# fusiyuan2010/CSC

Measured on AMD Instinct MI355X. Metric: encode MB/s (10^6 input bytes / wall-clock) on enwik9 stand-in, -m3 -d64m; stream bit-exact vs reference, higher is better.
Workload: dtype u8/u32 (byte + 32-bit integer work; 12-bit probabilities, 64-bit range-coder low)

## Files before the change

### csc_amd/csrc/csc_kernels.hip

```cpp
#include <hip/hip_runtime.h>
#include <stdint.h>
#include <stdlib.h>

#include "csc_device.h"
#include "csc_tables.h"

namespace cscmi {

#define DEV __device__ __forceinline__
#define GLOBAL_AS __attribute__((address_space(1)))
typedef GLOBAL_AS uint8_t gu8;
typedef GLOBAL_AS uint16_t gu16;
typedef GLOBAL_AS uint32_t gu32;
typedef uint32_t __attribute__((ext_vector_type(4))) raw_vec4;
typedef GLOBAL_AS raw_vec4 gvec4;
#define UNI(x) ((uint32_t)__builtin_amdgcn_readfirstlane((int)(x)))

#ifndef CSCMI_TU
#define CSCMI_TU 0
#endif
static __device__ __constant__ uint32_t d_p2bits[512];
static __device__ __constant__ uint32_t d_logtable[513];

__device__ static const uint32_t kDltIndex[5] = {1, 2, 3, 4, 8};
// ... 113 lines not shown
    c.ht2 = uni_gptr(c.ht2); c.ht3 = uni_gptr(c.ht3); c.ht6 = uni_gptr(c.ht6); c.bt_head = uni_gptr(c.bt_head); c.bt_nodes = uni_gptr(c.bt_nodes);
    c.p_lit = uni_gptr(c.p_lit); c.p_delta = uni_gptr(c.p_delta); c.mfbuf = uni_gptr(c.mfbuf);
    c.ht6_off = UNI(c.ht6_off); c.bth_off = UNI(c.bth_off);
    c.ht_bits = UNI(c.ht_bits); c.ht_width = UNI(c.ht_width); c.ht_low = UNI(c.ht_low); c.ht_cyc = UNI(c.ht_cyc);
    c.bt_bits = UNI(c.bt_bits); c.bt_size = UNI(c.bt_size); c.bt_cyc = UNI(c.bt_cyc); c.good_len = UNI(c.good_len);
    c.lz_good_len = UNI(c.lz_good_len); c.lz_bt_cyc = UNI(c.lz_bt_cyc); c.lz_ht_cyc = UNI(c.lz_ht_cyc);
    c.bt_pos = UNI(c.bt_pos); c.pos = UNI(c.pos); c.wnd_curpos = UNI(c.wnd_curpos);
    c.state = UNI(c.state); c.ctx = UNI(c.ctx); c.lp_rebuild_int = UNI(c.lp_rebuild_int);
    c.rc_low = uni64(c.rc_low); c.rc_range = UNI(c.rc_range); c.rc_cache = UNI(c.rc_cache); c.rc_cachesize = UNI(c.rc_cachesize);
    c.rc_size = UNI(c.rc_size); c.bc_size = UNI(c.bc_size); c.bc_curbits = UNI(c.bc_curbits); c.bc_curval = UNI(c.bc_curval); c.bsize = UNI(c.bsize);
    c.rc_buf = uni_gptr(c.rc_buf); c.bc_buf = uni_gptr(c.bc_buf); c.arena = uni_gptr(c.arena); c.swapbuf = uni_gptr(c.swapbuf);
    c.arena_used = UNI(c.arena_used); c.arena_cap = UNI(c.arena_cap); c.error = UNI(c.error);
    c.stage_base = UNI(c.stage_base); c.stage_end = UNI(c.stage_end);
    c.wv = UNI(c.wv); c.dp_seq = UNI(c.dp_seq); c.dp_idle = UNI(c.dp_idle); c.dp_seq_seen = UNI(c.dp_seq_seen);
    c.st_find = UNI(c.st_find); c.st_slide = UNI(c.st_slide); c.st_bt = UNI(c.st_bt); c.st_lit = UNI(c.st_lit); c.st_match = UNI(c.st_match);
    c.q_head = UNI(c.q_head); c.q_room = UNI(c.q_room);
}

DEV void wave_fence() { __builtin_amdgcn_fence(__ATOMIC_SEQ_CST, "workgroup"); }
DEV uint32_t rdlane(uint32_t v, uint32_t lane) { return (uint32_t)__builtin_amdgcn_readlane((int)v, (int)lane); }
DEV uint32_t wrlane(uint32_t val, uint32_t lane, uint32_t old) { return (threadIdx.x & 63u) == lane ? val : old; }

DEV uint64_t load8u(const gu8 *p)
{
    uintptr_t a = (uintptr_t)p;
    uint32_t sh = (uint32_t)a & 3u;
    const gu32 *q = (const gu32 *)(a & ~(uintptr_t)3);
    uint32_t d0 = q[0], d1 = q[1], d2 = q[2];
    uint32_t lo = __builtin_amdgcn_alignbyte(d1, d0, sh);
    uint32_t hi = __builtin_amdgcn_alignbyte(d2, d1, sh);
    return ((uint64_t)hi << 32) | lo;
}
DEV uint32_t ldb(const gu8 *p) { return UNI((uint32_t)*p); }

DEV uint64_t stage_load8(const uint32_t *stage, uint32_t byte_idx)
{
    uint32_t sh = byte_idx & 3u;
    const uint32_t *q = stage + (byte_idx >> 2);
    uint32_t d0 = q[0], d1 = q[1], d2 = q[2];
    uint32_t lo = __builtin_amdgcn_alignbyte(d1, d0, sh);
    uint32_t hi = __builtin_amdgcn_alignbyte(d2, d1, sh);
    return ((uint64_t)hi << 32) | lo;
}


__device__ __noinline__ void lanes_copy16(gvec4 *d4, const gvec4 *s4, uint32_t n16)
{
    for (uint32_t i = threadIdx.x & 63u; i < n16; i += 64) d4[i] = s4[i];
}
__device__ __noinline__ void lanes_copy8(gu8 *dst, const gu8 *src, uint32_t n)
{
    for (uint32_t t = threadIdx.x & 63u; t < n; t += 64) dst[t] = src[t];
}
__device__ __noinline__ void lanes_fill32(gu32 *dst, uint32_t n, uint32_t v)
{
    for (uint32_t t = threadIdx.x & 63u; t < n; t += 64) dst[t] = v;
}
__device__ __noinline__ void lanes_stage(uint8_t *sb, const gu8 *src, uint32_t first, uint32_t end)
{
    for (uint32_t t = first + (threadIdx.x & 63u); t < end; t += 64) sb[t] = src[t];
}
DEV void emit_block(Sc &c, uint32_t kind, const gu8 *buf, uint32_t size)
{
    uint32_t need = 16 + ((size + 15) & ~15u);
    if (c.arena_used + need > c.arena_cap) { c.error = ERR_ARENA_FULL; return; }
    gu8 *dst = c.arena + c.arena_used;
    wave_fence();
    ((gu32 *)dst)[0] = kind; ((gu32 *)dst)[1] = size;
    lanes_copy16((gvec4 *)(dst + 16), (const gvec4 *)buf, (size + 15) >> 4);
    c.arena_used += need;
}

constexpr uint32_t kCoderQ = 4096;
constexpr uint32_t kPDumpE = P_COUNT + 3;
struct CoderQ {
    uint32_t pub, tail, done, pad;
    uint32_t e[kCoderQ];
};
DEV void q_publish(Sc &c)
{
    __builtin_amdgcn_fence(__ATOMIC_RELEASE, "workgroup", "local");
    *(volatile __attribute__((address_space(3))) uint32_t *)&c.Q->pub = c.q_head;
}
constexpr uint32_t ERR_QUEUE_STALL = 0x40200000u;
DEV uint32_t q_wait_room(Sc &c, uint32_t need)
{
    uint32_t used, spins = 0;
    if (__builtin_expect(c.error != 0, 0)) return 0;
    while ((used = c.q_head - UNI(*(volatile __attribute__((address_space(3))) uint32_t *)&c.Q->tail)) > kCoderQ - need) {
        __builtin_amdgcn_s_sleep(2);
        if (++spins > (1u << 24)) { if (!c.error) c.error = ERR_QUEUE_STALL | (used & 0xFFFFu); return 0; }
    }
    return used;
}
DEV void q_push(Sc &c, uint32_t e)
{
    if (__builtin_expect(c.q_room == 0, 0)) {
        q_publish(c);
        c.q_room = umin(kCoderQ - 64u - q_wait_room(c, 128u), 256u);
    }
    c.Q->e[c.q_head & (kCoderQ - 1)] = e;
    c.q_head++; c.q_room--;
}

DEV void q_push_bits(Sc &c, uint32_t pold, uint32_t bit, uint32_t n, uint32_t from = 0)
{
    if (__builtin_expect(c.q_room < n, 0)) {
        q_publish(c);
        c.q_room = umin(kCoderQ - 64u - q_wait_room(c, 128u), 256u);
    }
    const uint32_t k = c.lane - from;
    c.Q->e[(c.q_head + (k < n ? k : 63u)) & (kCoderQ - 1)] = 0x80000000u | (bit ? 0x1000u : 0u) | pold;
    c.q_head += n; c.q_room -= n;
}

DEV void rc_put(Sc &c, uint32_t byte)
{
    c.rc_buf[c.rc_size++] = (uint8_t)byte;
    if (c.rc_size == c.bsize) { emit_block(c, 1, c.rc_buf, c.bsize); c.rc_size = 0; }
}

DEV void rc_shift_low(Sc &c)
{
    uint32_t low32 = (uint32_t)c.rc_low, top = (uint32_t)(c.rc_low >> 32);
    if (low32 < 0xFF000000u || top != 0) {
        uint32_t temp = c.rc_cache;
        do {
            rc_put(c, (temp + top) & 0xFF);
            temp = 0xFF;
        } while (--c.rc_cachesize != 0);
        c.rc_cache = low32 >> 24;
    }
    c.rc_cachesize++;
    c.rc_low = (uint64_t)(low32 << 8);
}

DEV void rc_code(Sc &c, uint32_t v, uint32_t p)
{
    if (c.Q) { q_push(c, 0x80000000u | (v ? 0x1000u : 0u) | p); return; }
    const uint32_t bound = (c.rc_range >> 12) * p;
    c.rc_low += v ? 0u : bound;
    c.rc_range = v ? bound : c.rc_range - bound;
    if (__builtin_expect(c.rc_range < (1u << 24), 0)) { c.rc_range <<= 8; rc_shift_low(c); }
}
DEV uint32_t p_update(uint32_t v, uint32_t p) { return v ? p + ((0xFFFu - p) >> 5) : p - (p >> 5); }

DEV void enc_bit_lds(Sc &c, uint32_t v, uint32_t idx)
{
    uint32_t p = UNI(c.L->P[idx]);
    c.L->P[idx] = p_update(v, p);
    rc_code(c, v, p);
}

DEV void bc_put(Sc &c, uint32_t byte)
{
    c.bc_buf[c.bc_size++] = (uint8_t)byte;
    if (c.bc_size == c.bsize) { emit_block(c, 0, c.bc_buf, c.bsize); c.bc_size = 0; }
}

DEV void enc_direct16(Sc &c, uint32_t val, uint32_t len)
{
    if (c.Q) { q_push(c, 0x40000000u | (len << 16) | (val & 0xFFFFu)); return; }
    c.bc_curval = (c.bc_curval << len) | val;
    c.bc_curbits += len;
    while (c.bc_curbits >= 8) {
        bc_put(c, (c.bc_curval >> (c.bc_curbits - 8)) & 0xFF);
// ... 412 lines not shown
```

### csc_amd/csrc/csc_kernels_dp4.inc

```

constexpr uint32_t kD4Rec = 256;
constexpr uint32_t kD4CandEnt = kD4Rec * 4;
constexpr uint32_t kD4RefEnt = 256;
constexpr uint32_t kD4Ent = kD4CandEnt + kD4RefEnt;
constexpr uint32_t kD4LA = 48;
constexpr uint32_t kD4Waves = 12;
DEV uint32_t d4_role(uint32_t w)
{
    constexpr uint32_t roles[12] = { 0, 6, 7, 1, 8, 5, 4, 2, 8, 8, 9, 3 };
    return w < 12 ? roles[w] : 8u;
}
constexpr uint32_t kD4Requested = 0xFFFFFFFFu;
#ifndef D4_IDLE_MUL
#define D4_IDLE_MUL 1
#endif
constexpr int kD4IdleSleep = 4 * D4_IDLE_MUL;
constexpr uint32_t kD4RefreshAt = 32;
constexpr uint32_t kD4MaxGood = 16;
constexpr uint32_t kD6Ring = 128;
constexpr uint32_t kD6MRing = 64;
constexpr uint32_t kD4MultiMax = 768;

struct Dp4X {
    uint32_t sb_seq, sb_ack, quit, abort;
    uint32_t sb0, pos0, size, gen;
    uint32_t m_pos;
    uint32_t m_ids[2];
    uint32_t ins_head;
    uint32_t cmp_next, cmp_pause, cmp_idle[3], cmp_cur[3];
    uint32_t ev_seq, ev_s, ev_len, ev_ack;
    uint32_t ref_head;
    uint32_t rq_head, rq_tail;
    uint32_t lit_req, lit_from, lit_done;
    uint32_t rid[4];
    uint32_t io_w0, io_gen, io_state0, io_lp_int, io_lit_seq, io_rq_head, io_wnd_lo, io_wnd_hi, io_wnd_size, io_vld, io_good, io_plit_lo, io_plit_hi;
    alignas(16) uint32_t o_kind, o_end, o_a0l, o_a0code, o_a0eid, o_a0slot, o_fin_i0, o_fin_i1, o_lp_int, o_lit_seq, o_rq_head, o_err;
#ifdef CSCMI_TIMERS
    uint32_t stat[8];
    uint32_t wtm[48];
#endif
    uint32_t rq[16][2];
    raw_vec4 cand[kD4Rec];
    uint8_t hflag[kD4Rec];
    uint32_t rec_tag[kD4Rec], rec_hsum[kD4Rec], rec_a0d[kD4Rec], rec_len[kD4Rec][16];
    uint32_t rec_m32[kD4Rec][16];
    raw_vec4 ent[kD4Ent];
    uint32_t fwd[kD4Ent];
    alignas(512) uint16_t litp[4][kD4Rec];
    alignas(16) uint16_t tab[64][32];
    alignas(256) raw_vec4 lab[16];
    alignas(512) uint32_t tent[2][16][8];
    alignas(256) raw_vec4 ver[16];
    uint32_t lab_seq, win_seq;
    alignas(16) uint32_t dump[8];
    alignas(8) uint32_t e_prog[2]; uint32_t e_stop[2];
#ifdef CSCMI_TIMERS
    uint32_t dbgp[64], dbgq[64][8], dbgl[32];
    uint32_t dbg;
    uint32_t tr_win, tr_lo, tr_hi;
#endif
    uint32_t lenp_new[32];
    uint32_t lt_pub, lt_done;
    uint32_t lt_rec[kD6Ring];
    uint32_t mt_pub, mt_done;
    uint32_t mt_rec[kD6MRing][2];
    uint32_t hS[2], h_reset, hand[20];
};
struct EncLds4 { EncLds base; Dp4X x; CoderQ q; };
__shared__ EncLds4 g_lds4;

DEV uint32_t d4_tag(uint32_t gen, uint32_t p) { return ((gen << 13) | p) + 1u; }
DEV Dp4X *d4x(Sc &c) { return reinterpret_cast<Dp4X *>(c.X); }

DEV uint32_t d4_eq4(uint32_t x)
{
    const uint32_t z = ~(((x & 0x7F7F7F7Fu) + 0x7F7F7F7Fu) | x) & 0x80808080u;
    return (((z >> 7) * 0x01020408u) >> 24) & 0xFu;
}
DEV uint32_t d4_eq8(uint64_t x) { return d4_eq4((uint32_t)x) | (d4_eq4((uint32_t)(x >> 32)) << 4); }

DEV bool d4_spin(Sc &c, Dp4X *X, uint32_t &spins, uint32_t site)
{
    __builtin_amdgcn_s_sleep(1);
    if ((++spins & 1023u) == 0 && (spins > (kDpSpinLimit << 2) || lds_vload(&X->abort))) {
        if (!lds_vload(&X->abort)) lds_vstore(&X->abort, 0x40000000u | (site << 16) | (c.wv << 24) | (spins & 0xFFFFu));
        c.error = lds_vload(&X->abort);
        return false;
    }
    return true;
}
template <int LANE> DEV uint32_t d4_wrlane(uint32_t old, uint32_t val)
{
    asm volatile("v_writelane_b32 %0, %1, %2" : "+v"(old) : "s"(val), "n"(LANE));
    return old;
}
DEV uint32_t umax_(uint32_t a, uint32_t b) { return a > b ? a : b; }
DEV uint32_t d4_parse_pos(Dp4X *X, uint32_t *ids0 = nullptr, uint32_t *ids1 = nullptr)
{
    typedef volatile __attribute__((address_space(3))) uint32_t vu32;
    typedef volatile __attribute__((address_space(3))) raw_vec4 vvec4;
    const uint32_t sq = UNI(*(vu32 *)&X->lab_seq);
    const uint32_t w0 = UNI(*(vu32 *)&X->io_w0), mp = UNI(*(vu32 *)&X->m_pos);
    const bool open = sq - 1u < 0xFFFFFFFEu;
    if (ids0) {
        const raw_vec4 lb = *(vvec4 *)&X->lab[(sq - 1u) & 15u];
        const uint32_t m0 = UNI(*(vu32 *)&X->m_ids[0]), m1 = UNI(*(vu32 *)&X->m_ids[1]);
        *ids0 = open ? UNI(lb.z) : m0; *ids1 = open ? UNI(lb.w) : m1;
    }
    return open ? umax_(mp, w0 + (sq < 2u ? 0u : sq - 2u)) : mp;
}
DEV uint32_t d4_rol1(uint32_t v) { return (uint32_t)__builtin_amdgcn_update_dpp(0, (int)v, 0x134, 0xF, 0xF, false); }


DEV void d4_insert_batch(Sc &c, Dp4X *X, uint32_t i0, uint32_t n, uint32_t &carry_h6)
{
    EncLds *L = c.L;
    const uint32_t lane = c.lane;
    const bool act = lane < n;
    const uint32_t sb0 = c.stage_base;
    const uint64_t v = stage_load8(L->stage, i0 + lane + 16);
    const uint32_t lo = (uint32_t)v, hi = (uint32_t)(v >> 32);
    const uint32_t h2 = hash2_of(lo), h3 = hash3_of(lo), h6 = hash6_mul(lo, hi) >> (32 - c.ht_bits);
// ... 1560 lines not shown
                L->fin2[k * 2u] = cD; L->fin2[k * 2u + 1u] = cBS;
#ifdef CSCMI_TIMERS
                if (k < 64) { X->dbgq[k][0] = cP; X->dbgq[k][5] = eP; X->dbgq[k][6] = 2; X->dbgq[k][7] = lp_int; }
#endif
                lds_fence();
                *(lds_vu32 *)&X->lab_seq = k + 1u;
            }
            vP = cP | vz; vD = cD | vz; vBS = cBS | vz; vI0 = cI0 | vz; vI1 = cI1 | vz; v_lp = lp_int | vz; v_reach = reach | vz;
            fI0 = cI0; fI1 = cI1;
            if (!out) pf_label();
#ifdef CSCMI_TIMERS
            t_gen += __builtin_readcyclecounter() - tg0;
#endif
            if (out) break;
        }
    }
#ifdef CSCMI_TIMERS
    const unsigned long long tse = __builtin_readcyclecounter();
    if (lane == 0) { atomicAdd(&X->wtm[13], (uint32_t)(tse - ts0) >> 4); atomicAdd(&X->wtm[14], n_straight); atomicAdd(&X->wtm[15], 1u);
        atomicAdd(&X->wtm[24], (uint32_t)(ts0 - tsp) >> 4); atomicAdd(&X->wtm[25], (uint32_t)t_first >> 4); atomicAdd(&X->wtm[26], (uint32_t)t_poll >> 4);
        atomicAdd(&X->wtm[27], (uint32_t)t_gen >> 4); atomicAdd(&X->wtm[28], n_gen); atomicAdd(&X->wtm[29], (uint32_t)(tse - t_last) >> 4); }
#endif
    lds_fence();
    *(lds_vu32 *)&X->lab_seq = kD5Stop;
    if (refreshed) { if (lane < 32) L->len_price[lane] = X->lenp_new[lane]; lds_fence(); }
    uint32_t f0 = kind == DP_EXIT_LIMIT ? fI0 : UNI(X->lab[end & 15u].z);
    uint32_t f1 = kind == DP_EXIT_LIMIT ? fI1 : UNI(X->lab[end & 15u].w);
    d5_forward_ids(X, lane, sel_rid, f0, f1);
    *(lds_vu32 *)&X->m_pos = w0 + end; *(lds_vu32 *)&X->m_ids[0] = f0; *(lds_vu32 *)&X->m_ids[1] = f1;
    {
        raw_vec4 o0, o1, o2;
        o0.x = kind; o0.y = end; o0.z = a0l; o0.w = a0code; o1.x = a0eid; o1.y = a0slot; o1.z = f0; o1.w = f1;
        o2.x = v_lp; o2.y = lit_seq; o2.z = rq_head; o2.w = err;
        *(lds_vvec4 *)&X->o_kind = o0; *(lds_vvec4 *)&X->o_a0eid = o1; *(lds_vvec4 *)&X->o_lp_int = o2;
    }
    lds_fence();
#ifdef CSCMI_TIMERS
    if (lane == 0) atomicAdd(&X->wtm[30], (uint32_t)(__builtin_readcyclecounter() - tse) >> 4);
#endif
}

DEV void d4_request(Sc &c, Dp4X *X, uint32_t id, uint32_t base, uint32_t &rq_head)
{
    if (rq_head - lds_vload(&X->rq_tail) >= 16u) return;
    X->rq[rq_head & 15u][0] = id;
    X->rq[rq_head & 15u][1] = base;
    X->fwd[id] = kD4Requested;
    rq_head++;
    lds_fence();
    lds_vstore(&X->rq_head, rq_head);
}

DEV bool d4_rebase_reps(Sc &c, Dp4X *X, uint32_t base, uint32_t &rq_head, bool wait)
{
    for (uint32_t r = 0; r < 4; r++) {
        const uint32_t id = lds_vload(&X->rid[r]);
        const uint32_t f = lds_vload(&X->fwd[id]);
        if (f == 0) {
            uint32_t spins = 0;
            while (rq_head - lds_vload(&X->rq_tail) >= 16u) if (!d4_spin(c, X, spins, 3)) return false;
            d4_request(c, X, id, base, rq_head);
        }
    }
    if (!wait) return true;
    for (uint32_t r = 0; r < 4; r++) {
        uint32_t id = lds_vload(&X->rid[r]);
        uint32_t spins = 0, f;
        while ((f = lds_vload(&X->fwd[id])) == kD4Requested) if (!d4_spin(c, X, spins, 4)) return false;
        if (f) { lds_fence(); X->rid[r] = f - 1; }
    }
    return true;
}


struct D6Cur { uint32_t lt_head, lt_seen, mt_head, mt_seen; };
DEV bool d6_join(Sc &c, Dp4X *X, D6Cur &q, bool lit_only = false);
DEV bool d6_room(Sc &c, Dp4X *X, uint32_t need, D6Cur &q)
{
    if (__builtin_expect(c.q_room < need, 0)) {
#ifdef CSCMI_TIMERS
        const uint64_t t0 = __builtin_readcyclecounter();
        const uint32_t out0 = (q.lt_head - lds_vload(&X->lt_done)) + (q.mt_head - lds_vload(&X->mt_done));
#endif
        if (!d6_join(c, X, q)) return false;
#ifdef CSCMI_TIMERS
        const uint64_t t1 = __builtin_readcyclecounter();
#endif
        q_publish(c);
        c.q_room = kCoderQ - 64u - q_wait_room(c, 64u + need);
#ifdef CSCMI_TIMERS
        if (c.lane == 0) { atomicAdd(&X->wtm[40], 1u); atomicAdd(&X->wtm[41], (uint32_t)(t1 - t0) >> 4); atomicAdd(&X->wtm[42], (uint32_t)(__builtin_readcyclecounter() - t1) >> 4); atomicAdd(&X->wtm[46], c.q_room >> 4);
                           atomicAdd(&X->wtm[31], out0); if (t1 - t0 < 2048u) atomicAdd(&X->wtm[47], 1u); }
#endif
    }
    return true;
}
DEV bool d6_literal(Sc &c, Dp4X *X, uint32_t sym, D6Cur &q)
{
    if (__builtin_expect(q.lt_head - q.lt_seen >= kD6Ring - 8u, 0)) {
        uint32_t spins = 0;
        while (q.lt_head - (q.lt_seen = lds_vload(&X->lt_done)) >= kD6Ring - 8u) if (!d4_spin(c, X, spins, 12)) return false;
    }
    const uint32_t fidx = P_STATE + c.state * 3;
    const uint32_t pold = c.L->P[fidx];
    c.L->P[fidx] = p_update(0, pold);
    c.Q->e[c.q_head & (kCoderQ - 1)] = 0x80000000u | pold;
    *(lds_vu32 *)&X->lt_rec[q.lt_head & (kD6Ring - 1)] = c.ctx | (sym << 8) | (c.q_head << 16);
    q.lt_head++;
    *(lds_vu32 *)&X->lt_pub = q.lt_head;
    c.q_head += 9; c.q_room -= 9;
    c.state = (c.state * 4) & 0x3F;
    c.ctx = sym;
    c.st_lit++;
    return true;
}
DEV void d6_flags(Sc &c, uint32_t nf, uint32_t idx, uint32_t bit)
{
    const bool on = c.lane < nf;
    const uint32_t i = on ? idx : kPDumpE;
    const uint32_t p = c.L->P[i];
    c.L->P[i] = p + (uint32_t)((int32_t)((bit ? 0xFFFu : 31u) - p) >> 5);
    c.Q->e[(c.q_head + (on ? c.lane : 63u)) & (kCoderQ - 1)] = 0x80000000u | (bit << 12) | p;
    c.q_head += nf; c.q_room -= nf;
}
DEV uint32_t d6_len_slots(uint32_t len) { return len < 8 ? 4u : len < 16 ? 5u : 9u; }
DEV bool d6_tree_record(Sc &c, Dp4X *X, uint32_t w0, uint32_t w1, uint32_t nslots, D6Cur &q)
{
    if (__builtin_expect(q.mt_head - q.mt_seen >= kD6MRing, 0)) {
        uint32_t spins = 0;
        while (q.mt_head - (q.mt_seen = lds_vload(&X->mt_done)) >= kD6MRing) if (!d4_spin(c, X, spins, 14)) return false;
    }
    *(lds_vu32 *)&X->mt_rec[q.mt_head & (kD6MRing - 1)][0] = w0 | (c.q_head << 16);
    *(lds_vu32 *)&X->mt_rec[q.mt_head & (kD6MRing - 1)][1] = w1;
    q.mt_head++;
    *(lds_vu32 *)&X->mt_pub = q.mt_head;
    c.q_head += nslots; c.q_room -= nslots;
    return true;
}
DEV bool d6_match(Sc &c, Dp4X *X, uint32_t dist, uint32_t len, D6Cur &q)
{
    d6_flags(c, 2, P_STATE + c.state * 3 + c.lane, 1u);
    const uint32_t sbits = len == 0 ? 3u : len <= 2 ? 4u : 5u;
    const uint32_t slot = dist_slot(dist), extra_bits = slot > 2 ? slot - 2 : 0;
    const uint32_t ndir = extra_bits > 4 ? (extra_bits - 4 > 16 ? 2u : 1u) : 0u;
    if (!d6_tree_record(c, X, 0u | (len << 1), dist, d6_len_slots(len) + sbits + ndir + (extra_bits ? 4u : 0u), q)) return false;
    c.state = (c.state * 4 + 1) & 0x3F;
    c.st_match++;
    return true;
}
DEV bool d6_rep_match(Sc &c, Dp4X *X, uint32_t rep_idx, uint32_t len, D6Cur &q)
{
    const uint32_t s3 = c.state * 3, k = c.lane;
    const uint32_t idx = k < 3 ? P_STATE + s3 + k : P_REPDIST + s3 - 1u + (k == 3 ? 1u : 2u | (rep_idx >> 1));
    const uint32_t bit = k < 3 ? (0x5u >> k) & 1u : (rep_idx >> ((4u - k) & 1u)) & 1u;
    d6_flags(c, 5, idx, bit);
    if (!d6_tree_record(c, X, 1u | (len << 1), 0u, d6_len_slots(len), q)) return false;
    c.state = (c.state * 4 + 3) & 0x3F;
    c.st_match++;
    return true;
}
DEV void d6_rep0len1(Sc &c)
{
    d6_flags(c, 3, P_STATE + c.state * 3 + c.lane, c.lane == 0 ? 1u : 0u);
    c.ctx = 0;
    c.state = (c.state * 4 + 2) & 0x3F;
    c.st_match++;
}
DEV bool d6_encode_nonlit(Sc &c, Dp4X *X, uint32_t ulen, uint32_t udist, D6Cur &q)
{
    EncLds *L = c.L;
    if (udist <= 4) {
        if (ulen == 1 && udist == 1) d6_rep0len1(c);
        else {
            if (!d6_rep_match(c, X, udist - 1, ulen - 2, q)) return false;
            uint32_t d = UNI(L->rep[udist - 1]);
// ... 3 lines not shown
    } else {
        if (!d6_match(c, X, udist - 5, ulen - 2, q)) return false;
        uint32_t r0 = UNI(L->rep[0]), r1 = UNI(L->rep[1]), r2 = UNI(L->rep[2]);
        L->rep[3] = r2; L->rep[2] = r1; L->rep[1] = r0; L->rep[0] = udist - 4;
    }
    return true;
}
DEV uint32_t d6_chunk_shape(uint32_t nd, uint32_t ql, bool on)
{
    const uint32_t len = ql & 0xFFFFu;
    const uint32_t kind = nd == 0 ? 0u : nd > 4 ? 1u : (nd == 1 && len == 1) ? 2u : 3u;
    const uint32_t l2 = len - 2u, dist = nd - 5u;
    const uint32_t sbits = l2 == 0 ? 3u : l2 <= 2 ? 4u : 5u;
    const uint32_t slot = dist_slot(dist), extra_bits = slot > 2 ? slot - 2 : 0;
    const uint32_t ndir = extra_bits > 4 ? (extra_bits - 4 > 16 ? 2u : 1u) : 0u;
    const uint32_t nf = kind == 0 ? 1u : kind == 1 ? 2u : kind == 2 ? 3u : 5u;
    const uint32_t tree = kind == 0 ? 8u : kind == 2 ? 0u : d6_len_slots(l2) + (kind == 1 ? sbits + ndir + (extra_bits ? 4u : 0u) : 0u);
    return on ? kind | (nf << 2) | ((nf + tree) << 8) : 0u;
}
DEV void d6_chunk_flag(bool act, uint32_t idx, uint32_t bit, uint32_t qslot, uint64_t same)
{
    const uint64_t am = __ballot(act);
    if (am == 0) return;
    const uint32_t lane = threadIdx.x & 63u;
    same &= am;
    const uint64_t below = same & ((1ull << lane) - 1ull), above = (same >> lane) >> 1;
    const uint32_t rank = (uint32_t)__builtin_popcountll(below);
    const uint32_t prev = below ? 63u - (uint32_t)__builtin_clzll(below) : lane;
    uint32_t pold = 0;
    if (act) pold = g_lds4.base.P[idx];
    uint32_t pnew = p_update(bit, pold);
    for (uint32_t d = 1; __ballot(act && rank >= d) != 0; d++) {
        const uint32_t v = (uint32_t)__builtin_amdgcn_ds_bpermute((int)(prev * 4u), (int)pnew);
        if (act && rank == d) { pold = v; pnew = p_update(bit, pold); }
    }
    if (act && above == 0) g_lds4.base.P[idx] = pnew;
    if (act) g_lds4.q.e[qslot & (kCoderQ - 1)] = 0x80000000u | (bit << 12) | pold;
}
__device__ __noinline__ uint32_t d6_chunk_lanes(uint32_t nd, uint32_t ql, uint32_t shape, uint32_t qpos, uint32_t n_, uint32_t state0_, uint32_t ctx0_, uint32_t lt_head_, uint32_t mt_head_)
{
    Dp4X *X = &g_lds4.x;
    const uint32_t lane = threadIdx.x & 63u;
    const uint32_t n = UNI(n_), state0 = UNI(state0_), ctx0 = UNI(ctx0_), lt_head = UNI(lt_head_), mt_head = UNI(mt_head_);
    const bool on = lane < n;
    const uint32_t kind = shape & 3u, nf = (shape >> 2) & 7u;
    const uint32_t len = ql & 0xFFFFu, last = ql >> 16;
    const uint64_t b0 = __ballot(on && (kind & 1u)), b1 = __ballot(on && (kind & 2u));
    const uint64_t h0 = (b0 << 3) | ((state0 & 1u) << 2) | (((state0 >> 2) & 1u) << 1) | ((state0 >> 4) & 1u);
    const uint64_t h1 = (b1 << 3) | (((state0 >> 1) & 1u) << 2) | (((state0 >> 3) & 1u) << 1) | ((state0 >> 5) & 1u);
    const uint32_t a = (uint32_t)(lane >= 3 ? b0 >> (lane - 3u) : h0 >> lane) & 7u, b = (uint32_t)(lane >= 3 ? b1 >> (lane - 3u) : h1 >> lane) & 7u;
    const uint32_t state = ((a >> 2) & 1u) | (((b >> 2) & 1u) << 1) | (((a >> 1) & 1u) << 2) | (((b >> 1) & 1u) << 3) | ((a & 1u) << 4) | ((b & 1u) << 5);
    const uint32_t before = (uint32_t)__shfl_up((int)last, 1);
    const uint32_t ctx = lane == 0 ? ctx0 : before;
    const bool is_lit = on && kind == 0, has_tree = on && (kind & 1u);
    const uint64_t lm = __ballot(is_lit), tm = __ballot(has_tree);
    if (is_lit) {
        const uint32_t r = __builtin_amdgcn_mbcnt_hi((uint32_t)(lm >> 32), __builtin_amdgcn_mbcnt_lo((uint32_t)lm, 0u));
        *(lds_vu32 *)&X->lt_rec[(lt_head + r) & (kD6Ring - 1)] = ctx | (last << 8) | (qpos << 16);
    }
    if (lm) lds_vstore(&X->lt_pub, lt_head + (uint32_t)__builtin_popcountll(lm));
    if (has_tree) {
        const uint32_t r = __builtin_amdgcn_mbcnt_hi((uint32_t)(tm >> 32), __builtin_amdgcn_mbcnt_lo((uint32_t)tm, 0u));
        *(lds_vu32 *)&X->mt_rec[(mt_head + r) & (kD6MRing - 1)][0] = (kind == 3 ? 1u : 0u) | ((len - 2u) << 1) | ((qpos + nf) << 16);
        *(lds_vu32 *)&X->mt_rec[(mt_head + r) & (kD6MRing - 1)][1] = kind == 1 ? nd - 5u : 0u;
    }
    if (tm) lds_vstore(&X->mt_pub, mt_head + (uint32_t)__builtin_popcountll(tm));
    uint64_t same = 0;
    for (uint64_t rem = __ballot(on); rem;) {
        const uint32_t sv = rdlane(state, (uint32_t)__builtin_ctzll(rem));
        const uint64_t mm = __ballot(on && state == sv);
        same = state == sv ? mm : same;
        rem &= ~mm;
    }
    const uint32_t s3 = state * 3u, rep_hi = ((nd - 1u) >> 1) & 1u;
    const bool is_rep = on && kind == 3;
    d6_chunk_flag(on, P_STATE + s3, kind != 0 ? 1u : 0u, qpos, same);
    d6_chunk_flag(on && kind != 0, P_STATE + s3 + 1u, kind == 1 ? 1u : 0u, qpos + 1u, same);
    d6_chunk_flag(on && kind >= 2, P_STATE + s3 + 2u, kind == 3 ? 1u : 0u, qpos + 2u, same);
    d6_chunk_flag(is_rep, P_REPDIST + s3, rep_hi, qpos + 3u, same);
    const uint64_t hi = __ballot(is_rep && rep_hi);
    d6_chunk_flag(is_rep, P_REPDIST + s3 + 1u + rep_hi, (nd - 1u) & 1u, qpos + 4u, same & (rep_hi ? hi : ~hi));
    return rdlane(((state * 4u + kind) & 0x3Fu) | (last << 8), n - 1u);
}
DEV bool d6_join(Sc &c, Dp4X *X, D6Cur &q, bool lit_only)
{
    uint32_t spins = 0;
    if (q.lt_seen != q.lt_head) {
        while ((q.lt_seen = lds_vload(&X->lt_done)) != q.lt_head) if (!d4_spin(c, X, spins, 13)) return false;
        dp_fence();
    }
    if (!lit_only && q.mt_seen != q.mt_head) {
        while ((q.mt_seen = lds_vload(&X->mt_done)) != q.mt_head) if (!d4_spin(c, X, spins, 15)) return false;
        lds_fence();
    }
    return true;
}
DEV void d6_trees(Sc &c)
{
    Dp4X *X = d4x(c);
    uint32_t done = 0, mdone = 0;
  for (;;) {
    uint32_t pub, mpub, idle = 0;
    for (;;) {
        pub = lds_vload(&X->lt_pub); mpub = lds_vload(&X->mt_pub);
        if (pub != done || mpub != mdone) break;
        if (lds_vload(&X->quit) || lds_vload(&X->abort)) return;
        if (idle < 48u) { idle++; __builtin_amdgcn_s_sleep(1 * D4_IDLE_MUL); }
        else __builtin_amdgcn_s_sleep(6 * D4_IDLE_MUL);
    }
    if (pub == done) {
        const uint32_t w0 = lds_vload(&X->mt_rec[mdone & (kD6MRing - 1)][0]), dist = lds_vload(&X->mt_rec[mdone & (kD6MRing - 1)][1]);
        const uint32_t len = (w0 >> 1) & 0xFFu, qpos = w0 >> 16;
        Decisions d; d.idx = 0; d.bit = 0; d.n = 0;
        dec_matchlen_1(c, d, len);
        uint32_t n_head = d.n, extra_bits = 0, extra_len = 0;
        if ((w0 & 1u) == 0) {
            uint32_t pdist_pos, sbits;
            if (len == 0) { pdist_pos = 0; sbits = 3; }
            else if (len <= 2) { pdist_pos = 16 * (len - 1) + 8; sbits = 4; }
            else if (len <= 5) { pdist_pos = 32 * (len - 3) + 8 + 16 * 2; sbits = 5; }
            else { pdist_pos = 32 * 3 + 8 + 16 * 2; sbits = 5; }
            const uint32_t slot = dist_slot(dist);
            extra_bits = slot > 2 ? slot - 2 : 0;
            dec_tree(c, d, P_DIST + pdist_pos, slot, sbits);
            n_head = d.n;
            if (extra_bits) {
                extra_len = dist - (1u << extra_bits) - 1;
                dec_tree(c, d, P_DIST_EXTRA + (extra_bits - 1) * 16, __brev(extra_len & 0x0Fu) >> 28, 4);
            }
        }
        const uint32_t pold = dec_apply(c, d);
        uint32_t ndir = 0;
        if (extra_bits > 4) {
            const uint32_t v = extra_len >> 4, l = extra_bits - 4;
            if (l <= 16) { g_lds4.q.e[(qpos + n_head) & (kCoderQ - 1)] = 0x40000000u | (l << 16) | (v & 0xFFFFu); ndir = 1; }
            else { g_lds4.q.e[(qpos + n_head) & (kCoderQ - 1)] = 0x40000000u | ((l - 16) << 16) | ((v >> 16) & 0xFFFFu);
                   g_lds4.q.e[(qpos + n_head + 1u) & (kCoderQ - 1)] = 0x40000000u | (16u << 16) | (v & 0xFFFFu); ndir = 2; }
        }
        {
            const uint32_t k = c.lane;
            const bool on = k < d.n;
            const uint32_t at = qpos + k + (k >= n_head ? ndir : 0u);
            lds_vu32 *const slot_p = on ? (lds_vu32 *)&g_lds4.q.e[at & (kCoderQ - 1)] : (lds_vu32 *)&g_lds4.q.pad;
            *slot_p = 0x80000000u | (d.bit << 12) | pold;
        }
        lds_fence();
        mdone++;
        lds_vstore(&X->mt_done, mdone);
    }
    while (done != pub) {
        const uint32_t nlit = umin(pub - done, 16u), n_a = umin(nlit, 8u), n_b = nlit - n_a;
        const uint32_t lane = c.lane, i = lane >> 3, k = lane & 7u;
        const uint32_t rec_a = *(lds_vu32 *)&X->lt_rec[(done + i) & (kD6Ring - 1)], rec_b = *(lds_vu32 *)&X->lt_rec[(done + 8u + i) & (kD6Ring - 1)];
        const uint32_t cc_a = ((rec_a >> 8) & 0xFFu) | 0x100u, cc_b = ((rec_b >> 8) & 0xFFu) | 0x100u;
        const uint32_t bit_a = (cc_a >> (7u - k)) & 1u, bit_b = (cc_b >> (7u - k)) & 1u;
        const bool act_a = i < n_a, act_b = i < n_b;
        const uint32_t cell_a = act_a ? (rec_a & 0xFFu) * 256u + (cc_a >> (8u - k)) : 0x80000000u | lane;
        const uint32_t cell_b = act_b ? (rec_b & 0xFFu) * 256u + (cc_b >> (8u - k)) : 0x80000040u | lane;
        uint32_t pold_a = 0, pold_b = 0;
        if (act_a) pold_a = c.p_lit[cell_a];
        if (act_b) pold_b = c.p_lit[cell_b];
        uint32_t prev_a = 0, prev_b = 0;
        bool later_a = false, later_b = false;
#pragma unroll
        for (uint32_t j = 7; j >= 1; j--) {
            const uint32_t o = (uint32_t)__builtin_amdgcn_ds_bpermute((int)((lane - 8u * j) * 4u), (int)cell_a);
            prev_a = (i >= j && o == cell_a) ? j : prev_a;
            const uint32_t o2 = (uint32_t)__builtin_amdgcn_ds_bpermute((int)((lane + 8u * j) * 4u), (int)cell_a);
            later_a = later_a || (i + j < 8u && o2 == cell_a);
        }
        uint32_t from_a = 0;
        if (n_b) {
#pragma unroll
            for (uint32_t j = 7; j >= 1; j--) {
                const uint32_t o = (uint32_t)__builtin_amdgcn_ds_bpermute((int)((lane - 8u * j) * 4u), (int)cell_b);
                prev_b = (i >= j && o == cell_b) ? j : prev_b;
                const uint32_t o2 = (uint32_t)__builtin_amdgcn_ds_bpermute((int)((lane + 8u * j) * 4u), (int)cell_b);
                later_b = later_b || (i + j < 8u && o2 == cell_b);
            }
#pragma unroll
            for (uint32_t j = 0; j < 8; j++) {
                const uint32_t r = (i + j) & 7u;
                const uint32_t oa = (uint32_t)__builtin_amdgcn_ds_bpermute((int)((lane + 8u * j) * 4u), (int)cell_a);
                from_a = (oa == cell_b && r + 1u > from_a) ? r + 1u : from_a;
                const uint32_t ob = (uint32_t)__builtin_amdgcn_ds_bpermute((int)((lane + 8u * j) * 4u), (int)cell_b);
                later_a = later_a || ob == cell_a;
            }
        }
        uint32_t pnew_a = p_update(bit_a, pold_a);
        const uint64_t cm_a = __ballot(prev_a != 0);
        if (__builtin_expect(cm_a != 0, 0)) {
            for (uint32_t r = 1; r < n_a; r++) {
                if (((cm_a >> (8u * r)) & 0xFFull) == 0) continue;
                const uint32_t v = (uint32_t)__builtin_amdgcn_ds_bpermute((int)((lane - 8u * prev_a) * 4u), (int)pnew_a);
                if (i == r && prev_a != 0) { pold_a = v; pnew_a = p_update(bit_a, pold_a); }
            }
        }
        if (n_b) {
            if (__ballot(from_a != 0)) {
                const uint32_t v = (uint32_t)__builtin_amdgcn_ds_bpermute((int)(((from_a - 1u) * 8u + k) * 4u), (int)pnew_a);
                pold_b = from_a ? v : pold_b;
            }
            uint32_t pnew_b = p_update(bit_b, pold_b);
            const uint64_t cm_b = __ballot(prev_b != 0);
            if (__builtin_expect(cm_b != 0, 0)) {
                for (uint32_t r = 1; r < n_b; r++) {
                    if (((cm_b >> (8u * r)) & 0xFFull) == 0) continue;
                    const uint32_t v = (uint32_t)__builtin_amdgcn_ds_bpermute((int)((lane - 8u * prev_b) * 4u), (int)pnew_b);
                    if (i == r && prev_b != 0) { pold_b = v; pnew_b = p_update(bit_b, pold_b); }
                }
            }
            if (act_b && !later_b) c.p_lit[cell_b] = pnew_b;
            if (act_b) g_lds4.q.e[((rec_b >> 16) + 1u + k) & (kCoderQ - 1)] = 0x80000000u | (bit_b << 12) | pold_b;
        }
        if (act_a && !later_a) c.p_lit[cell_a] = pnew_a;
        if (act_a) g_lds4.q.e[((rec_a >> 16) + 1u + k) & (kCoderQ - 1)] = 0x80000000u | (bit_a << 12) | pold_a;
        dp_fence();
        done += nlit;
        lds_vstore(&X->lt_done, done);
        pub = lds_vload(&X->lt_pub);
    }
  }
}

DEV void lz_compress_advanced_dp4(Sc &c, uint32_t size)
{
    EncLds *L = c.L;
    Dp4X *X = d4x(c);
    const uint32_t lane = c.lane;
    const uint32_t sb0 = c.wnd_curpos, pos0 = c.pos;
    uint32_t rq_head = lds_vload(&X->rq_head);
// ... 379 lines not shown
DEV void d4_worker(Sc &c);
__device__ __noinline__ void d4_worker_nl()
{
    Dp4X *X = &g_lds4.x;
    Sc c;
    const uint64_t sp = ((uint64_t)lds_vload(&X->hS[1]) << 32) | lds_vload(&X->hS[0]);
    sc_load_regs(c, (EncState *)(uintptr_t)sp, &g_lds4.base);
    c.X = X;
    if (lds_vload(&X->h_reset)) c.arena_used = 0;
    c.bt_head = nullptr; c.bt_nodes = nullptr; c.bt_bits = 0; c.bt_size = 0; c.gmb = 0; c.fast_ht = true; c.pair_ok = 0;
    c.wv = UNI(threadIdx.x >> 6);
    d4_worker(c);
}
DEV void d4_worker_call(Sc &) { d4_worker_nl(); }

DEV void d4_coder(Sc &c)
{
    CoderQ *Q = &g_lds4.q;
    Dp4X *X = d4x(c);
    uint32_t tail = 0;
    for (;;) {
        uint32_t pub;
        while ((pub = lds_vload(&Q->pub)) == tail) {
            if (lds_vload(&X->quit)) {
                EncState *S = c.S;
                if (c.lane == 0) {
                    S->rc_low = c.rc_low; S->rc_range = c.rc_range; S->rc_cache = c.rc_cache; S->rc_cachesize = c.rc_cachesize;
                    S->rc_size = c.rc_size; S->bc_size = c.bc_size; S->bc_curbits = c.bc_curbits; S->bc_curval = c.bc_curval;
                    S->arena_used = c.arena_used;
                    if (c.error) S->error = c.error;
                }
                return;
            }
            __builtin_amdgcn_s_sleep(2);
        }
        lds_acquire();
#ifdef CSCMI_TIMERS
        const uint64_t tc0 = __builtin_readcyclecounter();
        const uint32_t tail0 = tail;
#endif
        while (tail != pub) {
            const uint32_t n = umin(pub - tail, 64u);
            const uint32_t ev = Q->e[(tail + c.lane) & (kCoderQ - 1)];
            for (uint32_t j = 0; j < n; j++) {
                const uint32_t e = rdlane(ev, j);
                if (e & 0x80000000u) rc_code(c, (e >> 12) & 1u, e & 0xFFFu);
                else if (e & 0x40000000u) enc_direct16(c, e & 0xFFFFu, (e >> 16) & 0x1Fu);
                else coder_flush(c);
            }
            tail += n;
            lds_vstore(&Q->tail, tail);
        }
#ifdef CSCMI_TIMERS
        if (c.lane == 0) { atomicAdd(&X->wtm[43], (uint32_t)(__builtin_readcyclecounter() - tc0) >> 4); atomicAdd(&X->wtm[44], tail - tail0); atomicAdd(&X->wtm[45], 1u); }
#endif
    }
}

DEV void d4_worker(Sc &c)
{
    c.wv = d4_role(c.wv);
    if (c.wv == 8) return;
    if (c.wv == 1) d4_inserter(c);
    else if (c.wv == 9) d6_trees(c);
    else if (c.wv == 4) d4_service(c);
    else if (c.wv == 5) d4_coder(c);
    else if (c.wv >= 6) d5_edges(c, c.wv - 6u);
    else d4_compare(c, c.wv == 2 ? 0u : 1u);
}
DEV void d4_quit(Sc &c)
{
    Dp4X *X = d4x(c);
    if (c.Q) {
        q_publish(c);
        uint32_t spins = 0;
        while (lds_vload(&c.Q->tail) != c.q_head) if (!d4_spin(c, X, spins, 11)) break;
    }
    dp_fence();
    lds_vstore(&X->quit, 1);
    if (!c.error && lds_vload(&X->abort)) c.error = lds_vload(&X->abort);
#ifdef CSCMI_TIMERS
    for (int q = 2; q < 8; q++) c.tm[8 + q] += lds_vload(&X->stat[q]);
    if (g_lds4.x.dbgl[31] && c.S->stats.trace[61][0] == 0 && c.lane < 4 && g_lds4.x.dbgq[c.lane][2]) { unsigned long long *T = c.S->stats.trace[60]; T[12 * 0 + c.lane * 3 + 0] = g_lds4.x.dbgq[c.lane][0] + ((unsigned long long)g_lds4.x.dbgq[c.lane][4] << 32); T[c.lane * 3 + 1] = g_lds4.x.dbgq[c.lane][1] + ((unsigned long long)g_lds4.x.dbgq[c.lane][3] << 32); T[c.lane * 3 + 2] = g_lds4.x.dbgq[c.lane][2]; c.S->stats.trace[61][0] = 1; }
    if (c.lane == 0) for (int q = 0; q < 48; q++) atomicAdd((unsigned long long *)&c.S->stats.trace[q / 12][q % 12], (unsigned long long)lds_vload(&X->wtm[q]));
#endif
}
```

Baseline: 2.836.

## Batch up to four match records per wave and publish partial coder queue

The match-record worker now processes up to four (or two, for long records) match/distance bit-trees in parallel across lanes of one wave. Same-cell probability updates between records are chained via lane permutes so adaptive probabilities stay sequentially correct. Separately, when the producer runs out of queue room it no longer waits for all outstanding literal and match work. It publishes the queue head only up to the oldest unfinished record, then waits for room. This reduces serialization stalls but adds more per-lane index arithmetic and ordering subtlety.

Result: faster. 2.911, median of 6 (+2.7%).

```diff
diff --git a/csc_amd/csrc/csc_kernels.hip b/csc_amd/csrc/csc_kernels.hip
--- a/csc_amd/csrc/csc_kernels.hip
+++ b/csc_amd/csrc/csc_kernels.hip
@@ -219,6 +219,11 @@
     __builtin_amdgcn_fence(__ATOMIC_RELEASE, "workgroup", "local");
     *(volatile __attribute__((address_space(3))) uint32_t *)&c.Q->pub = c.q_head;
 }
+DEV void q_publish_to(Sc &c, uint32_t to)
+{
+    __builtin_amdgcn_fence(__ATOMIC_RELEASE, "workgroup", "local");
+    *(volatile __attribute__((address_space(3))) uint32_t *)&c.Q->pub = to;
+}
 constexpr uint32_t ERR_QUEUE_STALL = 0x40200000u;
 DEV uint32_t q_wait_room(Sc &c, uint32_t need)
 {
diff --git a/csc_amd/csrc/csc_kernels_dp4.inc b/csc_amd/csrc/csc_kernels_dp4.inc
--- a/csc_amd/csrc/csc_kernels_dp4.inc
+++ b/csc_amd/csrc/csc_kernels_dp4.inc
@@ -37,7 +37,7 @@
     alignas(16) uint32_t o_kind, o_end, o_a0l, o_a0code, o_a0eid, o_a0slot, o_fin_i0, o_fin_i1, o_lp_int, o_lit_seq, o_rq_head, o_err;
 #ifdef CSCMI_TIMERS
     uint32_t stat[8];
-    uint32_t wtm[48];
+    uint32_t wtm[52];
 #endif
     uint32_t rq[16][2];
     raw_vec4 cand[kD4Rec];
@@ -1764,15 +1764,26 @@
         const uint64_t t0 = __builtin_readcyclecounter();
         const uint32_t out0 = (q.lt_head - lds_vload(&X->lt_done)) + (q.mt_head - lds_vload(&X->mt_done));
 #endif
-        if (!d6_join(c, X, q)) return false;
+        const uint32_t ld = lds_vload(&X->lt_done), md = lds_vload(&X->mt_done);
+        uint32_t back = 0;
+        if (ld != q.lt_head) back = (c.q_head - (lds_vload(&X->lt_rec[ld & (kD6Ring - 1)]) >> 16)) & 0xFFFFu;
+        if (md != q.mt_head) back = max(back, (c.q_head - (lds_vload(&X->mt_rec[md & (kD6MRing - 1)][0]) >> 16)) & 0xFFFFu);
+        const bool all = back > kCoderQ - 64u - need;
+        if (all) { if (!d6_join(c, X, q)) return false; }
+        else lds_fence();
 #ifdef CSCMI_TIMERS
         const uint64_t t1 = __builtin_readcyclecounter();
 #endif
-        q_publish(c);
+        if (all) q_publish(c);
+        else {
+            const uint32_t last = lds_vload(&c.Q->pub), to = c.q_head - back;
+            q_publish_to(c, (int32_t)(to - last) < 0 ? last : to);
+        }
         c.q_room = kCoderQ - 64u - q_wait_room(c, 64u + need);
 #ifdef CSCMI_TIMERS
         if (c.lane == 0) { atomicAdd(&X->wtm[40], 1u); atomicAdd(&X->wtm[41], (uint32_t)(t1 - t0) >> 4); atomicAdd(&X->wtm[42], (uint32_t)(__builtin_readcyclecounter() - t1) >> 4); atomicAdd(&X->wtm[46], c.q_room >> 4);
-                           atomicAdd(&X->wtm[31], out0); if (t1 - t0 < 2048u) atomicAdd(&X->wtm[47], 1u); }
+                           atomicAdd(&X->wtm[31], out0); if (t1 - t0 < 2048u) atomicAdd(&X->wtm[47], 1u);
+                           atomicAdd(&X->wtm[22], all ? 1u : 0u); atomicAdd(&X->wtm[23], back); }
 #endif
     }
     return true;
@@ -1942,6 +1953,60 @@
     d6_chunk_flag(is_rep, P_REPDIST + s3 + 1u + rep_hi, (nd - 1u) & 1u, qpos + 4u, same & (rep_hi ? hi : ~hi));
     return rdlane(((state * 4u + kind) & 0x3Fu) | (last << 8), n - 1u);
 }
+struct D6Rec {
+    uint32_t len;
+    uint32_t k0[3], nb[3], x[3], base[3];
+    uint32_t n, n_head;
+    uint32_t ndir, dir0, dir1;
+};
+DEV D6Rec d6_rec(uint32_t w0, uint32_t dist)
+{
+    D6Rec r;
+    const uint32_t len = (w0 >> 1) & 0xFFu;
+    r.len = len;
+    r.k0[0] = len < 8 ? 1u : 2u; r.nb[0] = len < 16 ? 3u : 7u; r.x[0] = len < 8 ? len : len < 16 ? len - 8u : len - 16u;
+    r.base[0] = len < 8 ? (uint32_t)P_LEN_X1 : len < 16 ? (uint32_t)P_LEN_X2 : (uint32_t)P_LEN_X3;
+    uint32_t n = r.k0[0] + r.nb[0];
+    const bool match = (w0 & 1u) == 0;
+    const uint32_t sbits = len == 0 ? 3u : len <= 2 ? 4u : 5u;
+    const uint32_t pdist_pos = len == 0 ? 0u : len <= 2 ? 16u * (len - 1u) + 8u : 32u * (umin(len, 6u) - 3u) + 8u + 16u * 2u;
+    const uint32_t slot = dist_slot(dist), extra_bits = match && slot > 2 ? slot - 2u : 0u;
+    r.k0[1] = n; r.nb[1] = match ? sbits : 0u; r.x[1] = slot; r.base[1] = P_DIST + pdist_pos;
+    n += r.nb[1];
+    r.n_head = n;
+    const uint32_t extra_len = dist - (1u << (extra_bits & 31u)) - 1u;
+    r.k0[2] = n; r.nb[2] = extra_bits ? 4u : 0u; r.x[2] = __brev(extra_len & 0x0Fu) >> 28; r.base[2] = P_DIST_EXTRA + (extra_bits - 1u) * 16u;
+    n += r.nb[2];
+    r.n = n;
+    const uint32_t v = extra_len >> 4, l = extra_bits - 4u;
+    r.ndir = extra_bits > 4 ? (l > 16 ? 2u : 1u) : 0u;
+    r.dir0 = l <= 16 ? (l << 16) | (v & 0xFFFFu) : ((l - 16u) << 16) | ((v >> 16) & 0xFFFFu);
+    r.dir1 = (16u << 16) | (v & 0xFFFFu);
+    return r;
+}
+DEV void d6_rec_cell(const D6Rec &r, uint32_t k, uint32_t &idx, uint32_t &bit)
+{
+    idx = P_LEN_SLOT; bit = r.len >= 8 ? 1u : 0u;
+    if (k == 1 && r.len >= 8) { idx = P_LEN_SLOT + 1; bit = r.len >= 16 ? 1u : 0u; }
+#pragma unroll
+    for (uint32_t s = 0; s < 3; s++) {
+        const uint32_t l = k - r.k0[s];
+        if (l < r.nb[s]) { idx = r.base[s] + ((1u << l) | (r.x[s] >> ((r.nb[s] - l) & 31u))); bit = (r.x[s] >> ((r.nb[s] - 1u - l) & 31u)) & 1u; }
+    }
+}
+DEV uint32_t d6_rec_lane(const D6Rec &r, uint32_t idx)
+{
+    uint32_t k = 0xFFu;
+    if (idx == P_LEN_SLOT) k = 0;
+    if (idx == P_LEN_SLOT + 1 && r.len >= 8) k = 1;
+#pragma unroll
+    for (uint32_t s = 0; s < 3; s++) {
+        const uint32_t node = idx - r.base[s];
+        const uint32_t l = 31u - (uint32_t)__builtin_clz(node | 1u);
+        if (node >= 1u && node < (1u << r.nb[s]) && node == ((1u << l) | (r.x[s] >> ((r.nb[s] - l) & 31u)))) k = r.k0[s] + l;
+    }
+    return k;
+}
 DEV bool d6_join(Sc &c, Dp4X *X, D6Cur &q, bool lit_only)
 {
     uint32_t spins = 0;
@@ -1969,44 +2034,53 @@
         else __builtin_amdgcn_s_sleep(6 * D4_IDLE_MUL);
     }
     if (pub == done) {
-        const uint32_t w0 = lds_vload(&X->mt_rec[mdone & (kD6MRing - 1)][0]), dist = lds_vload(&X->mt_rec[mdone & (kD6MRing - 1)][1]);
-        const uint32_t len = (w0 >> 1) & 0xFFu, qpos = w0 >> 16;
-        Decisions d; d.idx = 0; d.bit = 0; d.n = 0;
-        dec_matchlen_1(c, d, len);
-        uint32_t n_head = d.n, extra_bits = 0, extra_len = 0;
-        if ((w0 & 1u) == 0) {
-            uint32_t pdist_pos, sbits;
-            if (len == 0) { pdist_pos = 0; sbits = 3; }
-            else if (len <= 2) { pdist_pos = 16 * (len - 1) + 8; sbits = 4; }
-            else if (len <= 5) { pdist_pos = 32 * (len - 3) + 8 + 16 * 2; sbits = 5; }
-            else { pdist_pos = 32 * 3 + 8 + 16 * 2; sbits = 5; }
-            const uint32_t slot = dist_slot(dist);
-            extra_bits = slot > 2 ? slot - 2 : 0;
-            dec_tree(c, d, P_DIST + pdist_pos, slot, sbits);
-            n_head = d.n;
-            if (extra_bits) {
-                extra_len = dist - (1u << extra_bits) - 1;
-                dec_tree(c, d, P_DIST_EXTRA + (extra_bits - 1) * 16, __brev(extra_len & 0x0Fu) >> 28, 4);
-            }
-        }
-        const uint32_t pold = dec_apply(c, d);
-        uint32_t ndir = 0;
-        if (extra_bits > 4) {
-            const uint32_t v = extra_len >> 4, l = extra_bits - 4;
-            if (l <= 16) { g_lds4.q.e[(qpos + n_head) & (kCoderQ - 1)] = 0x40000000u | (l << 16) | (v & 0xFFFFu); ndir = 1; }
-            else { g_lds4.q.e[(qpos + n_head) & (kCoderQ - 1)] = 0x40000000u | ((l - 16) << 16) | ((v >> 16) & 0xFFFFu);
-                   g_lds4.q.e[(qpos + n_head + 1u) & (kCoderQ - 1)] = 0x40000000u | (16u << 16) | (v & 0xFFFFu); ndir = 2; }
-        }
+        uint32_t n = umin(mpub - mdone, 4u), sh = 4;
+        const uint32_t lane = c.lane;
+        uint32_t w0 = *(lds_vu32 *)&X->mt_rec[(mdone + (lane >> 4)) & (kD6MRing - 1)][0], dist = *(lds_vu32 *)&X->mt_rec[(mdone + (lane >> 4)) & (kD6MRing - 1)][1];
+        D6Rec R = d6_rec(w0, dist);
+        if (__builtin_expect(__ballot((lane >> 4) < n && R.n > 14u) != 0, 0)) {
+            sh = 5; n = umin(n, 2u);
+            w0 = *(lds_vu32 *)&X->mt_rec[(mdone + (lane >> 5)) & (kD6MRing - 1)][0]; dist = *(lds_vu32 *)&X->mt_rec[(mdone + (lane >> 5)) & (kD6MRing - 1)][1];
+            R = d6_rec(w0, dist);
+        }
+        const uint32_t i = lane >> sh, k = lane & ((1u << sh) - 1u), qpos = w0 >> 16;
+        const bool on = i < n && k < R.n;
+        uint32_t idx, bit;
+        d6_rec_cell(R, k, idx, bit);
+        idx = on ? idx : 0xFFFFFFFFu;
+        uint32_t pold = c.L->P[on ? idx : kPDumpE];
+        uint32_t prev = lane, rank = 0;
+        bool later = false;
+        if (n > 1) {
+#pragma unroll
+            for (uint32_t j = 0; j < 4; j++) {
+                if (j >= n) break;
+                const D6Rec Rj = d6_rec(rdlane(w0, j << sh), rdlane(dist, j << sh));
+                const uint32_t kj = d6_rec_lane(Rj, idx);
+                const bool hit = kj != 0xFFu;
+                if (hit && j < i) { prev = (j << sh) + kj; rank++; }
+                later = later || (hit && j > i);
+            }
+        }
+        uint32_t pnew = p_update(bit, pold);
+        for (uint32_t d = 1; d < n && __ballot(rank >= d) != 0; d++) {
+            const uint32_t v = (uint32_t)__builtin_amdgcn_ds_bpermute((int)(prev * 4u), (int)pnew);
+            if (rank == d) { pold = v; pnew = p_update(bit, pold); }
+        }
+        c.L->P[on && !later ? idx : kPDumpE] = pnew;
         {
-            const uint32_t k = c.lane;
-            const bool on = k < d.n;
-            const uint32_t at = qpos + k + (k >= n_head ? ndir : 0u);
-            lds_vu32 *const slot_p = on ? (lds_vu32 *)&g_lds4.q.e[at & (kCoderQ - 1)] : (lds_vu32 *)&g_lds4.q.pad;
-            *slot_p = 0x80000000u | (d.bit << 12) | pold;
+            const uint32_t kd = k - ((1u << sh) - 2u);
+            const bool dir = i < n && kd < R.ndir;
+            const uint32_t at = dir ? qpos + R.n_head + kd : qpos + k + (k >= R.n_head ? R.ndir : 0u);
+            lds_vu32 *const slot_p = on || dir ? (lds_vu32 *)&g_lds4.q.e[at & (kCoderQ - 1)] : (lds_vu32 *)&g_lds4.q.pad;
+            *slot_p = dir ? 0x40000000u | (kd ? R.dir1 : R.dir0) : 0x80000000u | (bit << 12) | pold;
         }
         lds_fence();
-        mdone++;
+        mdone += n;
         lds_vstore(&X->mt_done, mdone);
+#ifdef CSCMI_TIMERS
+        if (lane == 0) { atomicAdd(&X->wtm[48], 1u); atomicAdd(&X->wtm[49], n); }
+#endif
     }
     while (done != pub) {
         const uint32_t nlit = umin(pub - done, 16u), n_a = umin(nlit, 8u), n_b = nlit - n_a;
@@ -2552,6 +2626,6 @@
 #ifdef CSCMI_TIMERS
     for (int q = 2; q < 8; q++) c.tm[8 + q] += lds_vload(&X->stat[q]);
     if (g_lds4.x.dbgl[31] && c.S->stats.trace[61][0] == 0 && c.lane < 4 && g_lds4.x.dbgq[c.lane][2]) { unsigned long long *T = c.S->stats.trace[60]; T[12 * 0 + c.lane * 3 + 0] = g_lds4.x.dbgq[c.lane][0] + ((unsigned long long)g_lds4.x.dbgq[c.lane][4] << 32); T[c.lane * 3 + 1] = g_lds4.x.dbgq[c.lane][1] + ((unsigned long long)g_lds4.x.dbgq[c.lane][3] << 32); T[c.lane * 3 + 2] = g_lds4.x.dbgq[c.lane][2]; c.S->stats.trace[61][0] = 1; }
-    if (c.lane == 0) for (int q = 0; q < 48; q++) atomicAdd((unsigned long long *)&c.S->stats.trace[q / 12][q % 12], (unsigned long long)lds_vload(&X->wtm[q]));
-#endif
-}
+    if (c.lane == 0) for (int q = 0; q < 52; q++) atomicAdd((unsigned long long *)&c.S->stats.trace[q / 12][q % 12], (unsigned long long)lds_vload(&X->wtm[q]));
+#endif
+}
```
